# nmichlo/mtg-vision

Measured on AMD Instinct MI355X. Metric: cards/sec end-to-end (detect+embed+top-1 over 100k bank), 640x640, higher is better.
Workload: dtype f32 (products as 3 x f16 MFMA on hi/lo-split operands, f32 accumulate)

## Files before the change

### mtg-vision_amd/csrc/gemm_f32.hip

```cpp
#include "gemm_kernel.h"
#include "gemm_sp.h"
#include "operand_registry.h"

#include <stdlib.h>
#include <string.h>
#include <algorithm>
#include <string>
#include <vector>

namespace mtgv {

GemmArgs linear_args(const float* A, int lda, const float* W, const float* bias, float* Out, int ldo, int M, int N, int K,
                     int act) {
  GemmArgs a;
  a.A = A;
  a.W = W;
  a.Out = Out;
  a.bias = bias;
  a.M = M, a.N = N, a.K = K;
  a.c_total = lda;
  a.Cin = K;
  a.ldo = ldo;
  a.act = act;
  return a;
}

GemmArgs conv_args(const ConvIn& in, const float* W, const float* bias, int cout, int kh, int kw, int stride, int pad,
                   const ConvOut& out, int act) {
  GemmArgs a;
  a.A = in.p, a.a_fmt = in.fmt;
  a.W = W;
  a.bias = bias;
  a.Out = out.p, a.out_fmt = out.fmt;
  a.M = in.n * out.h * out.w, a.N = cout, a.K = kh * kw * in.c;
  a.H = in.h, a.Wd = in.w, a.c_total = in.ct, a.c_off = in.co, a.Cin = in.c;
  a.KH = kh, a.KW = kw, a.stride = stride, a.pad = pad;
  a.OH = out.h, a.OW = out.w, a.OH2 = out.h, a.OW2 = out.w;
  a.ldo = out.ct, a.o_off = out.co;
  a.act = act;
  return a;
}

bool gemm_dispatch_f32(const GemmDev& g, const GemmPlan& pl, bool conv, bool apro, int grid, hipStream_t s) {
  return gemm_dispatch<0>(g, pl, conv, apro, grid, s);
}
bool gemm_dispatch_f16x3(const GemmDev& g, const GemmPlan& pl, bool conv, bool apro, int grid, hipStream_t s);


namespace {
struct GemmProf {
  bool on = false;
  std::vector<hipEvent_t> ev;
  size_t used = 0;
  double flops = 0;
  double bytes = 0;
  long launches = 0;
  struct Rec { int M, N, K, KH, stride, batch, act, apro, grn, topk, tm, tn, bk, sp; double bytes, fill, xflops; };
  std::vector<Rec> recs;
} g_prof;
}

void gemm_profile_enable(bool on) {
  g_prof.on = on;
  g_prof.used = 0;
  g_prof.flops = 0;
  g_prof.bytes = 0;
  g_prof.launches = 0;
  g_prof.recs.clear();
}

void gemm_profile_dump(const char* path) {
  FILE* f = fopen(path, "w");
  MTGV_CHECK(f != nullptr, ERR_RUNTIME, "cannot open %s", path);
  fprintf(f, "idx,M,N,K,KH,stride,batch,act,apro,grn,topk,tm,tn,bk,ms,tflops,bytes,sp,fill,xflops\n");
  for (size_t i = 0; i + 1 < g_prof.used && i / 2 < g_prof.recs.size(); i += 2) {
    HIP_OK(hipEventSynchronize(g_prof.ev[i + 1]));
    float t = 0.f;
    HIP_OK(hipEventElapsedTime(&t, g_prof.ev[i], g_prof.ev[i + 1]));
    const auto& r = g_prof.recs[i / 2];
    const double fl = 2.0 * r.M * r.N * r.K * r.batch + r.xflops;
    fprintf(f, "%zu,%d,%d,%d,%d,%d,%d,%d,%d,%d,%d,%d,%d,%d,%.4f,%.2f,%.0f,%d,%.0f,%.0f\n", i / 2, r.M, r.N, r.K, r.KH, r.stride, r.batch, r.act,
            r.apro, r.grn, r.topk, r.tm, r.tn, r.bk, t, fl / (t * 1e-3) / 1e12, r.bytes, r.sp, r.fill, r.xflops);
  }
  fclose(f);
  gemm_sp_stamps_dump((std::string(path) + ".stamps").c_str());
}

bool gemm_profile_enabled() { return g_prof.on; }
double gemm_profile_bytes() { return g_prof.bytes; }

void gemm_profile_read(double* ms, double* flops, long* launches) {
  double total = 0;
  for (size_t i = 0; i + 1 < g_prof.used; i += 2) {
    HIP_OK(hipEventSynchronize(g_prof.ev[i + 1]));
    float t = 0.f;
    HIP_OK(hipEventElapsedTime(&t, g_prof.ev[i], g_prof.ev[i + 1]));
    total += t;
  }
  if (ms) *ms = total;
  if (flops) *flops = g_prof.flops;
  if (launches) *launches = g_prof.launches;
}

static void prof_begin(const GemmArgs& a, const GemmPlan& pl, hipStream_t s, int sp, double fill, double bytes_override = -1.0,
                       double xflops = 0.0) {
  if (!g_prof.on) return;
  while (g_prof.ev.size() < g_prof.used + 2) {
    hipEvent_t e;
    HIP_OK(hipEventCreate(&e));
    g_prof.ev.push_back(e);
  }
  HIP_OK(hipEventRecord(g_prof.ev[g_prof.used], s));
  const double xfl = (a.W2 != nullptr ? 2.0 * (double)a.M * a.N2 * a.N : 0.0) + xflops;
  g_prof.flops += 2.0 * (double)a.M * a.N * a.K * a.batch + xfl;
  {
    const double a_el = is_conv(a) ? (double)(a.M / (a.OH * a.OW)) * a.H * a.Wd * a.Cin : (double)a.M * a.K;
    const double w_el = (double)a.N * a.K;
    const double o_el = a.topk > 0 ? (double)a.M * ceil_div(a.N, 64) * a.topk * 2
                                   : (a.W2 != nullptr ? (double)a.M * a.N2 + (double)a.N2 * a.N : (double)a.M * a.N);
    const double r_el = a.res != nullptr ? (double)a.M * a.N : 0.0;
    double by = 4.0 * ((a.strideA != 0 || a.batch == 1 ? a.batch : 1) * a_el + (a.strideW != 0 || a.batch == 1 ? a.batch : 1) * w_el +
                       a.batch * (o_el + r_el));
    if (bytes_override >= 0.0) by = bytes_override;
    g_prof.bytes += by;
    g_prof.recs.push_back({a.M, a.N, a.K, a.KH, a.stride, a.batch, a.act, a.a_scale != nullptr, a.grn_part != nullptr, a.topk,
                           pl.tm, pl.tn, pl.bk, sp, by, fill, xfl});
  }
  g_prof.launches += 1;
}
static void prof_end(hipStream_t s) {
  if (!g_prof.on) return;
  HIP_OK(hipEventRecord(g_prof.ev[g_prof.used + 1], s));
  g_prof.used += 2;
}

static int g_prec = -1;

int gemm_precision() {
  if (g_prec < 0) {
    const char* e = getenv("MTGV_GEMM_PREC");
    if (e == nullptr || !*e || !strcmp(e, "f16x3")) g_prec = GEMM_PREC_F16X3;
    else if (!strcmp(e, "f32")) g_prec = GEMM_PREC_F32;
    else MTGV_CHECK(false, ERR_INVALID, "MTGV_GEMM_PREC=%s: expected f32 or f16x3", e);
  }
  return g_prec;
}

void gemm_set_precision(int prec) {
  MTGV_CHECK(prec == GEMM_PREC_F32 || prec == GEMM_PREC_F16X3, ERR_INVALID, "gemm precision %d: 0 (f32) or 1 (f16x3)", prec);
  g_prec = prec;
}

static GemmPlan tile(int tm, int tn, int bk, int M, int N) {
  GemmPlan pl{tm, tn, bk, 0, 0};
  pl.tiles_m = ceil_div(M, pl.bm());
  pl.tiles_n = ceil_div(N, pl.bn());
  return pl;
}

static GemmPlan gemm_plan(int M, int N, int K, bool heavy_epilogue, bool scaled_a) {
  if (const char* e = getenv("MTGV_GEMM_TILE")) {
    int tm = 0, tn = 0, bk = 0;
    if (sscanf(e, "%d,%d,%d", &tm, &tn, &bk) == 3 && (tm == 1 || tm == 2) && tn >= 1 && tn <= 5 && (bk == 16 || bk == 32))
      return tile(tm, tn, bk, M, N);
  }
  const bool split = gemm_precision() == GEMM_PREC_F16X3;
  const double ov = 36.0 + (heavy_epilogue ? 48.0 : 0.0);
  static const double eff_tab[2][3][6] = {
      {{0, 0.88, 0.93, 1.00, 0.80, 0.62},
       {0, 0.85, 0.93, 0.98, 1.00, 0.85},
       {0, 0.80, 0.90, 1.00, 0.85, 0.80}},
      {{0, 0.65, 0.88, 1.00, 0.90, 0.72},
       {0, 0.62, 0.90, 0.97, 1.00, 0.90},
       {0, 0.65, 0.88, 1.00, 0.88, 0.70}}};
  const double* eff = eff_tab[split ? 1 : 0][scaled_a ? 2 : heavy_epilogue ? 1 : 0];
  int best_tn = 1;
  double best = -1;
  const long tiles_m = ceil_div(M, 128);
  for (int tn = 1; tn <= 5; ++tn) {
// ... 29 lines not shown
  if (gemm_sp_topk_layout(a, slots, cols)) return;
  const GemmPlan pl = plan_for(a);
  *slots = pl.tiles_n;
  *cols = pl.bn();
}

size_t gemm_grn_part_floats_max(int M, int N, int hw) {
  size_t mx = 0;
  for (int unit : {32, 64, 128, 256}) {
    const size_t f = (size_t)ceil_div(M, unit) * ((unit - 1) / hw + 2) * N;
    mx = f > mx ? f : mx;
  }
  return mx;
}

static bool ln_fusable(const GemmArgs& a, const GemmPlan& pl) {
  if (!(pl.tm == 1 && pl.tn == 3 && pl.bk == 16 && is_conv(a) && a.N == pl.bn() && a.M % pl.bm() == 0)) return false;
  if (a.batch != 1 || a.act != ACT_NONE || a.res != nullptr || a.a_scale != nullptr || a.grn_part != nullptr || a.topk > 0 ||
      a.crop_boxes != nullptr || a.m_count != nullptr || is_remap(a) || a.out_fmt != 0 || a.a_fmt != 0)
    return false;
  GemmArgs t = a;
  t.ln_w = nullptr;
  return gemm_sp_plan(t).cfg < 0;
}

bool gemm_ln_fusable(const GemmArgs& a) { return ln_fusable(a, plan_for(a)); }

void gemm_launch(const GemmArgs& args, hipStream_t s) {
  GemmArgs a = args;
  const GemmPlan pl = plan_for(a);
  if (a.ln_w != nullptr)
    MTGV_CHECK(a.ln_b != nullptr && ln_fusable(a, pl), ERR_INVALID, "gemm: this launch cannot normalise its rows in the epilogue");
  MTGV_CHECK(a.batch >= 1 && a.batch <= 65535, ERR_INVALID, "gemm: batch=%d", a.batch);
  MTGV_CHECK(a.M > 0 && a.N > 0 && a.K > 0, ERR_INVALID, "gemm: empty problem M=%d N=%d K=%d", a.M, a.N, a.K);
  MTGV_CHECK(a.K % 4 == 0 && a.Cin % 4 == 0 && a.c_total % 4 == 0 && a.c_off % 4 == 0, ERR_INVALID,
             "gemm: K=%d Cin=%d c_total=%d c_off=%d must be multiples of 4", a.K, a.Cin, a.c_total, a.c_off);
  MTGV_CHECK(a.K == a.KH * a.KW * a.Cin, ERR_INVALID, "gemm: K=%d != %d*%d*%d", a.K, a.KH, a.KW, a.Cin);
  MTGV_CHECK(((uintptr_t)a.A % 16) == 0 && ((uintptr_t)a.W % 16) == 0, ERR_INVALID, "gemm: operands must be 16-byte aligned");
  MTGV_CHECK((long)a.M * (long)(a.OH * a.OW > a.hw ? a.OH * a.OW : a.hw) < (1l << 40), ERR_INVALID, "gemm: M too large for fastdiv");
  const bool conv = is_conv(a);
  const bool apro = a.a_scale != nullptr;
  MTGV_CHECK(!(apro && conv), ERR_INVALID, "gemm: GRN prologue only on 1x1");
  MTGV_CHECK(!(apro && a.act != ACT_NONE), ERR_INVALID, "gemm: GRN prologue is only combined with a linear epilogue");
  MTGV_CHECK(a.a_shift == nullptr, ERR_INVALID, "gemm: fold the GRN shift into the bias (fold_shift_into_bias_launch)");
  if (!conv) MTGV_CHECK(a.OH == a.H && a.OW == a.Wd, ERR_INVALID, "gemm: 1x1 geometry mismatch");
  if (apro || a.grn_part) MTGV_CHECK(a.hw > 0 && a.M % a.hw == 0, ERR_INVALID, "gemm: hw=%d must divide M=%d", a.hw, a.M);
  const SpPlan sp = gemm_sp_plan(a);
  if (a.grn_part) {
    const GrnLayout l = grn_layout(a, sp, pl);
    a.segmax = l.segmax;
    a.grn_unit_rows = l.unit_rows;
  }
  if (sp.cfg >= 0) {
    prof_begin(a, pl, s, 1, g_prof.on ? gemm_sp_fill_bytes(a, sp) : 0.0, -1.0, a.xflops);
    gemm_sp_launch(a, sp, s);
    prof_end(s);
    return;
  }

  MTGV_CHECK(a.os_nq == 0, ERR_INVALID, "gemm: the grouped scatter epilogue (os_nq) exists on the LDS-DMA kernel only");
  MTGV_CHECK(a.W2 == nullptr, ERR_INVALID, "gemm: the chained 1x1 exists on the LDS-DMA kernel only");
  MTGV_CHECK(conv_pad_h(a) == a.pad && conv_pad_w(a) == a.pad && a.bias_tab == nullptr, ERR_INVALID,
             "gemm: asymmetric padding and the bias table exist on the LDS-DMA kernel only");
  GemmDev g;
  g.a = a;
  if (gemm_precision() == GEMM_PREC_F16X3 && g.a.W_split == nullptr && a.strideW == 0)
    g.a.W_split = operand_split(a.W, a.K, &g.a.wscale);
  if (gemm_precision() != GEMM_PREC_F16X3) g.a.W_split = nullptr, g.a.wscale = nullptr;
  g.d_ohw = make_fastdiv((uint32_t)(a.OH * a.OW));
  g.d_ow = make_fastdiv((uint32_t)a.OW);
  g.d_cin = make_fastdiv((uint32_t)a.Cin);
  g.d_kwcin = make_fastdiv((uint32_t)(a.KW * a.Cin));
  g.d_hw = make_fastdiv((uint32_t)(a.hw > 0 ? a.hw : 1));
  g.d_cw = make_fastdiv((uint32_t)(a.crop_w > 0 ? a.crop_w : 1));
  g.tiles_m = pl.tiles_m;
  g.tiles_n = pl.tiles_n;
  g.nseg_max = a.hw > 0 ? std::min(pl.bm(), (pl.bm() - 1) / a.hw + 2) : 1;
  {
    const double lim = 4294967296.0 - 65536.0;
    const double a_bytes = (double)a.M * a.c_total * 4.0 + (double)a.c_off * 4.0, w_bytes = (double)a.N * a.K * 4.0;
    const double s_bytes = a.a_scale != nullptr && a.hw > 0 ? (double)(a.M / a.hw) * a.K * 4.0 : 0.0;
    g.off32_ok = a_bytes < lim && w_bytes < lim && s_bytes < lim;
  }
  g.remap = is_remap(a);
  const int grid = pl.tiles_m * pl.tiles_n;

  if (a.topk > 0) {
    MTGV_CHECK(!conv && !apro, ERR_INVALID, "gemm: top-k epilogue needs the 128x64x16 tile");
    MTGV_CHECK(a.cand_s != nullptr && a.cand_i != nullptr && a.topk <= 128, ERR_INVALID, "gemm: bad top-k arguments");
  }
  prof_begin(a, pl, s, 0, (double)grid * a.batch * (pl.bm() + pl.bn()) * a.K * 4.0);
  const bool found = gemm_precision() == GEMM_PREC_F16X3 ? gemm_dispatch_f16x3(g, pl, conv, apro, grid, s)
                                                         : gemm_dispatch_f32(g, pl, conv, apro, grid, s);
  if (found) {
    HIP_OK(hipGetLastError());
    prof_end(s);
    return;
  }
  MTGV_CHECK(false, ERR_INVALID, "gemm: no kernel for tile tm=%d tn=%d bk=%d", pl.tm, pl.tn, pl.bk);
}

__global__ __launch_bounds__(256) void grn_finalize_kernel(const float* __restrict__ part, int bm, int segmax, int hw, int N,
                                                          FastDiv d_hw, FastDiv d_bm, const float* __restrict__ gamma,
                                                          float* __restrict__ scale) {
  extern __shared__ __attribute__((aligned(16))) float sm[];
  float* gx = sm;
  float* red = sm + N;
// ... 59 lines not shown
```

### mtg-vision_amd/csrc/gemm_sp.hip

```cpp
#include "gemm_sp.h"

#include <limits.h>
#include <array>
#include <mutex>
#include <utility>
#include <vector>

#include "gemm_sp_kernel.h"
#include "operand_registry.h"

namespace mtgv {

__global__ __launch_bounds__(256) void sp8_pack_plain_kernel(const float* __restrict__ in, sp_h8* __restrict__ out, long n8) {
  const long i = (long)blockIdx.x * 256 + threadIdx.x;
  if (i >= n8) return;
  sp_h8 hi, lo;
  sp8_split8(*reinterpret_cast<const sp_f4*>(in + i * 8), *reinterpret_cast<const sp_f4*>(in + i * 8 + 4), hi, lo);
  out[2 * i] = hi;
  out[2 * i + 1] = lo;
}

void sp8_pack_plain_launch(const float* in, void* out, long rows, int K, hipStream_t s) {
  MTGV_CHECK(K % 8 == 0, ERR_INVALID, "sp8: K=%d must be a multiple of 8", K);
  const long n8 = rows * (K / 8);
  if (n8 <= 0) return;
  hipLaunchKernelGGL(sp8_pack_plain_kernel, dim3((unsigned)((n8 + 255) / 256)), dim3(256), 0, s, in, (sp_h8*)out, n8);
  HIP_OK(hipGetLastError());
}

const char* sp_zero_page() {
  static char* zero[MTGV_MAX_DEVICES] = {};
  static std::mutex mu;
  const int dev = current_device();
  std::lock_guard<std::mutex> lk(mu);
  if (zero[dev] == nullptr) {
    HIP_OK(hipMalloc((void**)&zero[dev], 256));
    HIP_OK(hipMemset(zero[dev], 0, 256));
  }
  return zero[dev];
}

template <int ID>
void gemm_sp_launch_cfg(const SpDev& g, int amode, hipStream_t s);

namespace {
typedef void (*SpLaunchFn)(const SpDev&, int, hipStream_t);
template <int... ID>
constexpr std::array<SpLaunchFn, sizeof...(ID)> sp_launchers(std::integer_sequence<int, ID...>) {
  return {{&gemm_sp_launch_cfg<ID>...}};
}
const auto kLaunch = sp_launchers(std::make_integer_sequence<int, kSpNumCfg>{});

const double kEff[kSpNumCfg] = {0.93, 1.00, 0.88, 0.80, 0.62, 0.00, 0.00, 0.00};

SpPlan plan_of(int cfg, int M, int N) {
  const SpTile& k = kSpTile[cfg];
  SpPlan pl;
  pl.cfg = cfg, pl.bm = k.bm(), pl.bn = k.bn(), pl.unit_rows = k.wave_rows();
  pl.tiles_m = ceil_div(M, k.bm()), pl.tiles_n = ceil_div(N, k.bn());
  return pl;
}
}

bool window_conv_on() {
  static const bool on = env_int("MTGV_SP_WINDOW", 1) != 0;
  return on;
}

bool window_conv_fits(const GemmArgs& a, const SpPlan& pl) {
  const SpTile& k = kSpTile[pl.cfg];
  if (!(window_conv_on() && a.KH == 3 && a.KW == 3 && a.stride == 1 && conv_pad_h(a) == 1 && conv_pad_w(a) == 1 && a.stride_w <= 0 && a.Cin % k.kps() == 0 &&
        a.OH == a.H && a.OW == a.Wd))
    return false;
  return sp_window_fits(k, a.Wd);
}

static bool n160_instance(const GemmArgs& a) {
  SpPlan p;
  p.cfg = SP_CFG_N160;
  return is_conv(a) && a.a_fmt == 1 && a.W2 == nullptr && a.act == ACT_SILU && a.out_fmt == 1 && a.res == nullptr && a.grn_part == nullptr &&
         !is_remap(a) && a.topk == 0 && window_conv_fits(a, p);
}

bool gemm_sp_active() { return gemm_precision() == GEMM_PREC_F16X3; }

bool gemm_sp_takes_sp8(const float* W, int M, int N, int K, int lda, int c_off) {
  if (!gemm_sp_active()) return false;
  if (K % 8 != 0 || N % 4 != 0 || lda % 8 != 0 || c_off % 8 != 0 || M <= 0) return false;
  return operand_sp8(W, K, nullptr, nullptr);
}

static int chain_cfg(const GemmArgs& a) {
  if (a.W2 == nullptr || a.Out2 == nullptr || !is_conv(a)) return -1;
  if (!(gemm_sp_active() && a.a_fmt == 1 && a.act == ACT_SILU && a.res == nullptr && a.grn_part == nullptr && a.topk == 0 && a.batch == 1 &&
        a.os_nq == 0 && a.a_scale == nullptr && a.ln_w == nullptr))
    return -1;
  if (a.bias_tab == nullptr) {
    if (!(a.os == 1 && a.OH2 == a.OH && a.OW2 == a.OW)) return -1;
  } else {
    if (!(a.bias == nullptr && a.os >= 1 && a.oy >= 0 && a.oy < a.os && a.ox >= 0 && a.ox < a.os && a.OH2 == a.OH * a.os && a.OW2 == a.OW * a.os &&
          ((uintptr_t)a.bias_tab & 15) == 0))
      return -1;
    SpPlan p;
    p.cfg = sp_chain_cfg(a.N);
    if (p.cfg < 0 || window_conv_fits(a, p)) return -1;
  }
  if (sp_chain_cfg(a.N) < 0 || a.N2 <= 0 || a.N2 % 32 != 0 || a.N2 > a.N) return -1;
  if (a.K % 8 != 0 || a.c_total % 8 != 0 || a.c_off % 8 != 0 || a.ldo2 % 4 != 0 || a.o_off2 % 4 != 0 || ((uintptr_t)a.Out2 & 15) != 0) return -1;
  if (a.out_fmt2 == 1 && (a.ldo2 % 8 != 0 || a.o_off2 % 8 != 0)) return -1;
  if (a.stride_w > 0 || a.Cin % 8 != 0) return -1;
  if (!operand_sp8(a.W, a.K, nullptr, nullptr) || !operand_sp8(a.W2, a.N, nullptr, nullptr)) return -1;
  return sp_chain_cfg(a.N);
}
bool gemm_sp_chain_ok(const GemmArgs& a) { return chain_cfg(a) >= 0; }

SpPlan gemm_sp_plan(const GemmArgs& a) {
  SpPlan pl;
  if (a.W2 != nullptr) {
    const int c = chain_cfg(a);
    MTGV_CHECK(c >= 0, ERR_INVALID, "gemm: this launch cannot chain its second layer (M=%d N=%d K=%d N2=%d): ask gemm_sp_chain_ok first", a.M,
               a.N, a.K, a.N2);
    return plan_of(c, a.M, a.N);
  }
  const bool sp8_in = a.a_fmt == 1;
  auto none = [&]() -> SpPlan {
    MTGV_CHECK(!sp8_in && a.out_fmt == 0 && a.res_fmt == 0, ERR_INVALID,
               "gemm: SP8 tensors handed to a launch the SP kernel cannot run (M=%d N=%d K=%d)", a.M, a.N, a.K);
    return pl;
  };
  if (!gemm_sp_active()) return none();
  const bool conv = is_conv(a);
  const bool remap = is_remap(a);
  if (a.batch != 1 || a.crop_boxes != nullptr || a.m_count != nullptr || a.ln_w != nullptr) return none();
  if (a.topk > 0) {
    const SpTile& k1 = kSpTile[SP_CFG_TOPK];
    if (sp8_in || conv || a.K % 8 != 0 || a.c_total % 8 != 0 || a.c_off % 8 != 0 || ((uintptr_t)a.A & 15) != 0 || a.a_scale != nullptr ||
        a.a_mul != 1.0f || a.res != nullptr || a.act != ACT_NONE || a.M < k1.bm() || a.N < k1.bn() || !operand_sp8(a.W, a.K, nullptr, nullptr))
      return none();
    return plan_of(SP_CFG_TOPK, a.M, a.N);
  }
  if (conv && (!sp8_in || a.stride_w > 0 || a.Cin % 8 != 0)) return none();
  if (remap && !sp8_in) return none();
  if (a.K % 8 != 0 || a.c_total % 8 != 0 || a.c_off % 8 != 0 || a.ldo % 4 != 0 || a.o_off % 4 != 0 ||
      (a.res != nullptr && a.ldr % 4 != 0))
    return none();
  if (a.N % 4 != 0 && (a.out_fmt != 0 || a.res != nullptr || a.grn_part != nullptr || remap)) return none();
  if (a.out_fmt == 1 && (a.N % 8 != 0 || a.ldo % 8 != 0 || a.o_off % 8 != 0 || a.grn_part != nullptr)) return none();
  if (a.res != nullptr && a.res_fmt == 1 && (a.ldr % 8 != 0 || a.N % 8 != 0)) return none();
  if (((uintptr_t)a.Out % 16) != 0 || (a.res != nullptr && ((uintptr_t)a.res % 16) != 0)) return none();
  if (sp8_in && a.a_scale != nullptr) return none();
  if (!operand_sp8(a.W, a.K, nullptr, nullptr)) return none();
  if (!sp8_in && (a.N < 64 || a.M < 128)) return none();

  int best = -1;
  double best_cost = 0;
  const int force = env_int("MTGV_SP_CFG", INT_MIN);
  const bool forced = force != INT_MIN;
  if (forced && force >= 0 && force < kSpNumCfg && kSpTile[force].ks == 2 && (force != SP_CFG_N160 || n160_instance(a))) best = force;
  if (best < 0) {
    for (int c = 0; c < kSpNumCfg; ++c) {
      const SpTile& k = kSpTile[c];
      if (kEff[c] <= 0.0) continue;
      if (!sp8_in && a.a_scale != nullptr && sp_ring(k, SP_A_F32_MUL, kSpRing) > kSpTwoPerCu) continue;
      const long tiles = (long)ceil_div(a.M, k.bm()) * ceil_div(a.N, k.bn());
      const double rounds = (double)((tiles + kSpRoundTiles - 1) / kSpRoundTiles);
      const double per_cu = rounds * 2.0 * k.bm() * k.bn();
      const double cost = per_cu / kEff[c];
      if (best < 0 || cost < best_cost) best = c, best_cost = cost;
    }
  }
  if (a.os_nq == kSpTile[SP_CFG_OS_NQ].bn() && !forced) best = SP_CFG_OS_NQ;
  {
    SpPlan p16;
    p16.cfg = SP_CFG_WIN16;
    if (!forced && conv && sp8_in && a.Cin % kSpTile[best].kps() != 0 && a.N <= kSpTile[SP_CFG_WIN16].bn() && window_conv_fits(a, p16))
      best = SP_CFG_WIN16;
  }
  if (!forced && a.N == kSpTile[SP_CFG_N160].bn() && n160_instance(a) && ceil_div(a.M, kSpTile[SP_CFG_N160].bm()) > kSpRoundTiles &&
      env_int("MTGV_DET_HEAD_DIRECT", 1) != 0)
    best = SP_CFG_N160;
  if (best == SP_CFG_TOPK && !conv && sp8_in && a.grn_part != nullptr && a.topk == 0 && a.K >= 256 && a.M >= 12288) best = SP_CFG_PW1_8W;
  return plan_of(best, a.M, a.N);
}

namespace {
struct StampRec { int M, N, K, cfg, amode, act, tiles; long* buf; };
std::vector<StampRec> g_stamps;
bool stamps_on() {
  static const bool on = env_int("MTGV_SP_STAMPS", 0) != 0;
  return on;
}
}

bool gemm_sp_topk_layout(const GemmArgs& a, int* slots, int* cols) {
  const SpPlan pl = gemm_sp_plan(a);
  if (pl.cfg < 0) return false;
  const SpTile& k = kSpTile[pl.cfg];
  *slots = pl.tiles_n * k.wn;
  *cols = k.wave_cols();
  return true;
}

double gemm_sp_fill_bytes(const GemmArgs& a, const SpPlan& pl) {
  const SpTile& k = kSpTile[pl.cfg];
  const double tiles = (double)pl.tiles_m * pl.tiles_n;
  const double b_tile = (double)k.bn() * a.K * 4.0;
  double a_tile = (double)k.bm() * a.K * 4.0;
  if (a.a_fmt == 1 && is_conv(a) && window_conv_fits(a, pl)) a_tile = (double)sp_window_bytes(k, a.Wd) * (a.Cin / k.kps());
  if (a.a_scale != nullptr) a_tile += (double)(a.K / k.kps()) * sp_stage_mul(SP_A_F32_MUL);
  return tiles * (a_tile + b_tile);
}

void gemm_sp_stamps_dump(const char* path) {
  if (g_stamps.empty()) return;
  HIP_OK(hipDeviceSynchronize());
  FILE* f = fopen(path, "wb");
  MTGV_CHECK(f != nullptr, ERR_RUNTIME, "cannot open %s", path);
  std::vector<long> host;
  for (const StampRec& r : g_stamps) {
    const int hdr[8] = {r.M, r.N, r.K, r.cfg, r.amode, r.act, r.tiles, 0};
    fwrite(hdr, sizeof(int), 8, f);
    host.resize((size_t)r.tiles * 8);
    HIP_OK(hipMemcpy(host.data(), r.buf, host.size() * sizeof(long), hipMemcpyDeviceToHost));
    fwrite(host.data(), sizeof(long), host.size(), f);
    HIP_OK(hipFree(r.buf));
  }
  fclose(f);
  g_stamps.clear();
}

int gemm_sp_topk_hi16_range_cols() { return kSpTile[SP_CFG_TOPK].wave_cols(); }
int gemm_sp_topk_hi16_slots(int N) { return ceil_div(N, kSpTile[SP_CFG_TOPK].bn()) * kSpTile[SP_CFG_TOPK].wn; }

// ... 107 lines not shown
```

### mtg-vision_amd/csrc/gemm_sp_cfg.h

```cpp
#pragma once
#include <stddef.h>

namespace mtgv {

struct SpTile {
  int wm, wn, tm, tn, ks;
  constexpr int bm() const { return 32 * tm * wm; }
  constexpr int bn() const { return 32 * tn * wn; }
  constexpr int rb() const { return 64 * ks; }
  constexpr int kps() const { return 16 * ks; }
  constexpr int waves() const { return wm * wn; }
  constexpr int wave_rows() const { return 32 * tm; }
  constexpr int wave_cols() const { return 32 * tn; }
};

constexpr SpTile kSpTile[] = {
    {2, 2, 2, 2, 2},
    {2, 2, 2, 3, 2},
    {4, 1, 1, 3, 2},
    {4, 1, 1, 2, 2},
    {4, 1, 1, 1, 2},
    {4, 2, 1, 3, 2},
    {4, 1, 1, 1, 1},
    {4, 1, 1, 5, 2},
};
constexpr int kSpNumCfg = sizeof(kSpTile) / sizeof(kSpTile[0]);

enum SpCfgId : int {
  SP_CFG_TOPK = 1,
  SP_CFG_OS_NQ = 3,
  SP_CFG_PW1_8W = 5,
  SP_CFG_WIN16 = 6,
  SP_CFG_N160 = 7,
};
static_assert(kSpTile[SP_CFG_PW1_8W].bm() == kSpTile[SP_CFG_TOPK].bm() && kSpTile[SP_CFG_PW1_8W].bn() == kSpTile[SP_CFG_TOPK].bn(),
              "the eight-wave twin covers the same block");
static_assert(kSpTile[SP_CFG_WIN16].ks == 1 && kSpTile[SP_CFG_OS_NQ].bn() == 64 && kSpTile[SP_CFG_N160].bn() == 160, "named configurations");

constexpr bool sp_tile_chains(const SpTile& t) { return t.wn == 1 && t.tm == 1 && t.ks == 2 && t.tn <= 3; }
constexpr int sp_chain_cfg(int N) {
  for (int c = 0; c < kSpNumCfg; ++c)
    if (sp_tile_chains(kSpTile[c]) && kSpTile[c].bn() == N) return c;
  return -1;
}
constexpr int sp_chain_max_n() {
  int n = 0;
  for (int c = 0; c < kSpNumCfg; ++c)
    if (sp_tile_chains(kSpTile[c]) && kSpTile[c].bn() > n) n = kSpTile[c].bn();
  return n;
}

enum SpAMode : int {
  SP_A_SP8 = 0,
  SP_A_REG = 1,
  SP_A_CONV = 2,
  SP_A_F32_MUL = 3,
  SP_A_F32 = 4,
  SP_A_WINDOW = 5,
  SP_A_HI16 = 6,
};
enum SpEpi : int {
  SP_EPI_ARGS = -1,
  SP_EPI_F32 = 0,
  SP_EPI_SP8_OUT = 1,
  SP_EPI_RES_F32 = 2,
  SP_EPI_RES_SP8 = 4,
  SP_EPI_GRN = 8,
  SP_EPI_TOPK = 16,
  SP_EPI_CHAIN = 32,
  SP_EPI_CHAIN_PHASE = 96,
};
constexpr bool sp_epi_chains(int epi) { return epi == SP_EPI_CHAIN || epi == SP_EPI_CHAIN_PHASE; }
constexpr int SP_ACT_ARGS = -1;

constexpr int kSpPiece = 1024;
constexpr int kSpSlab = 32 * 128;
constexpr int kSpRing = 2;
constexpr int kSpDeepRing = 4;
constexpr long kSpRoundTiles = 512;

constexpr int sp_stage_a(const SpTile& t, int amode) { return amode == SP_A_WINDOW ? 0 : t.bm() * t.rb(); }
constexpr int sp_stage_b(const SpTile& t) { return t.bn() * t.rb(); }
constexpr int sp_stage_mul(int amode) { return amode == SP_A_F32_MUL ? kSpPiece : 0; }
constexpr int sp_stage(const SpTile& t, int amode) { return sp_stage_a(t, amode) + sp_stage_b(t) + sp_stage_mul(amode); }
constexpr size_t sp_ring(const SpTile& t, int amode, int nst) { return (size_t)nst * sp_stage(t, amode); }

constexpr int sp_window_px(int bm, int rb, int Wd) {
  const int rpp = kSpPiece / rb;
  return (bm + 2 * Wd + 2 + rpp - 1) / rpp * rpp;
}
constexpr size_t sp_window_bytes(const SpTile& t, int Wd) { return (size_t)sp_window_px(t.bm(), t.rb(), Wd) * t.rb(); }

constexpr int sp_staging_wave(const SpTile& t) { return 32 * 128 * t.tn; }
constexpr int sp_staging_rounds(const SpTile& t, int amode, int nst) {
  return (amode != SP_A_WINDOW && (size_t)t.waves() * sp_staging_wave(t) > sp_ring(t, amode, nst)) ? 2 : 1;
}

constexpr int sp_chain_a2(const SpTile& t) { return t.waves() * kSpSlab; }
constexpr int sp_chain_w2(const SpTile& t) { return t.waves() * kSpSlab * (1 + t.tn); }
constexpr size_t sp_chain_bytes(const SpTile& t, int N2) { return (size_t)sp_chain_w2(t) + (size_t)t.tn * N2 * 128; }

constexpr size_t sp_launch_lds(const SpTile& t, int amode, int epi, int nst, int Wd) {
  size_t lds = sp_ring(t, amode, nst);
  if (amode == SP_A_WINDOW) {
    const size_t win = sp_window_bytes(t, Wd) + lds, stage = (size_t)t.waves() * sp_staging_wave(t);
    lds = win > stage ? win : stage;
  }
  if (sp_epi_chains(epi) && lds < sp_chain_bytes(t, sp_chain_max_n())) lds = sp_chain_bytes(t, sp_chain_max_n());
  return lds;
}

constexpr size_t kSpTwoPerCu = 80 * 1024;
constexpr bool sp_window_fits(const SpTile& t, int Wd) {
  return sp_window_bytes(t, Wd) + sp_ring(t, SP_A_WINDOW, kSpRing) <= kSpTwoPerCu;
}
constexpr int sp_window_ring(const SpTile& t, int Wd, long tiles) {
  return (tiles <= kSpRoundTiles && sp_window_bytes(t, Wd) + sp_ring(t, SP_A_WINDOW, kSpDeepRing) <= kSpTwoPerCu) ? kSpDeepRing : kSpRing;
}
constexpr bool sp_window_ring_deepens(const SpTile& t) { return sp_window_ring(t, 1, 1) == kSpDeepRing; }
static_assert(sp_window_fits(kSpTile[SP_CFG_N160], 80) && !sp_window_ring_deepens(kSpTile[SP_CFG_N160]) &&
                  sp_launch_lds(kSpTile[SP_CFG_N160], SP_A_WINDOW, SP_EPI_SP8_OUT, kSpRing, 80) <= kSpTwoPerCu,
              "the 128 x 160 tile runs two blocks per CU");

}
```

### mtg-vision_amd/csrc/gemm_sp_inst.h

```cpp
#pragma once
#include "gemm_sp_kernel.h"

namespace mtgv {

namespace {
template <int ID, int AMODE, int ACT, int EPI, int NST = kSpRing>
void sp_launch_one(const SpDev& g, hipStream_t s) {
  constexpr SpTile T = kSpTile[ID];
  if constexpr (AMODE == SP_A_WINDOW && NST == kSpRing && sp_window_ring_deepens(T)) {
    if (sp_window_ring(T, g.Wd, (long)g.tiles_m * g.tiles_n) == kSpDeepRing) return sp_launch_one<ID, AMODE, ACT, EPI, kSpDeepRing>(g, s);
  }
  const size_t lds = sp_launch_lds(T, AMODE, EPI, NST, g.Wd);
  constexpr auto kern = gemm_sp_kernel<T.wm, T.wn, T.tm, T.tn, T.ks, NST, AMODE, ACT, EPI>;
  lds_opt_in<kern>(lds, (AMODE == SP_A_WINDOW || sp_epi_chains(EPI)) ? 160 * 1024 : (int)lds);
  hipLaunchKernelGGL(kern, dim3((unsigned)(g.tiles_m * g.tiles_n)), dim3(64 * T.waves()), lds, s, g);
}

template <int ID, int AMODE, int ACT>
void sp_pick(const SpDev& g, int epi, hipStream_t s) {
  MTGV_CHECK(!sp_epi_chains(epi), ERR_RUNTIME, "gemm_sp: no chained-1x1 instance for A mode %d in configuration %d", AMODE, ID);
  sp_launch_one<ID, AMODE, ACT, SP_EPI_ARGS>(g, s);
}
template <int ID, int AMODE, int ACT, int E0, int... ES>
void sp_pick(const SpDev& g, int epi, hipStream_t s) {
  if (epi == E0) sp_launch_one<ID, AMODE, ACT, E0>(g, s);
  else sp_pick<ID, AMODE, ACT, ES...>(g, epi, s);
}

constexpr int SP8_RES = SP_EPI_SP8_OUT | SP_EPI_RES_SP8;

template <int ID, int AMODE>
void sp_pick_conv(const SpDev& g, int epi, hipStream_t s) {
  if (g.act != ACT_SILU) sp_pick<ID, AMODE, SP_ACT_ARGS>(g, epi, s);
  else if constexpr (sp_tile_chains(kSpTile[ID]) && AMODE == SP_A_CONV)
    sp_pick<ID, AMODE, ACT_SILU, SP_EPI_SP8_OUT, SP8_RES, SP_EPI_CHAIN, SP_EPI_CHAIN_PHASE>(g, epi, s);
  else if constexpr (sp_tile_chains(kSpTile[ID])) sp_pick<ID, AMODE, ACT_SILU, SP_EPI_SP8_OUT, SP8_RES, SP_EPI_CHAIN>(g, epi, s);
  else sp_pick<ID, AMODE, ACT_SILU, SP_EPI_SP8_OUT, SP8_RES>(g, epi, s);
}
}

template <int ID>
void gemm_sp_launch_cfg(const SpDev& g, int amode, hipStream_t s);

#if SP_CFG_ID == 7
static_assert(SP_CFG_ID == SP_CFG_N160, "the single-instance configuration");
template <>
void gemm_sp_launch_cfg<SP_CFG_N160>(const SpDev& g, int amode, hipStream_t s) {
  MTGV_CHECK(amode == SP_A_WINDOW && g.act == ACT_SILU && g.topk == 0 && sp_epi_of(g) == SP_EPI_SP8_OUT, ERR_RUNTIME,
             "gemm_sp: configuration %d runs SiLU window convs with SP8 output only (A mode %d, act %d)", (int)SP_CFG_N160, amode, g.act);
  sp_launch_one<SP_CFG_N160, SP_A_WINDOW, ACT_SILU, SP_EPI_SP8_OUT>(g, s);
}
#endif

template <int ID>
void gemm_sp_launch_cfg(const SpDev& g, int amode, hipStream_t s) {
  constexpr SpTile T = kSpTile[ID];
  if (g.topk > 0) {
    if constexpr (ID == SP_CFG_TOPK) {
      MTGV_CHECK((amode == SP_A_F32 || amode == SP_A_HI16) && g.act == ACT_NONE, ERR_INVALID, "gemm_sp: top-k needs aligned f32 queries");
      if (amode == SP_A_HI16) sp_launch_one<ID, SP_A_HI16, ACT_NONE, SP_EPI_TOPK>(g, s);
      else sp_launch_one<ID, SP_A_F32, ACT_NONE, SP_EPI_TOPK>(g, s);
      return;
    } else {
      MTGV_CHECK(false, ERR_INVALID, "gemm_sp: no top-k instance in this configuration");
    }
  }
  const int epi = sp_epi_of(g);
  if constexpr (T.ks != 2) {
    MTGV_CHECK(amode == SP_A_WINDOW || amode == SP_A_CONV, ERR_RUNTIME, "gemm_sp: configuration %d runs convolutions only (A mode %d)", ID, amode);
    if (amode == SP_A_WINDOW) sp_pick_conv<ID, SP_A_WINDOW>(g, epi, s);
    else sp_pick_conv<ID, SP_A_CONV>(g, epi, s);
  } else if (amode == SP_A_SP8) {
    switch (g.act) {
      case ACT_NONE: sp_pick<ID, SP_A_SP8, ACT_NONE, SP_EPI_F32, SP_EPI_SP8_OUT>(g, epi, s); break;
      case ACT_MISH: sp_pick<ID, SP_A_SP8, ACT_MISH, SP_EPI_GRN>(g, epi, s); break;
      case ACT_GELU: sp_pick<ID, SP_A_SP8, ACT_GELU, SP_EPI_GRN>(g, epi, s); break;
      case ACT_SILU: sp_pick<ID, SP_A_SP8, ACT_SILU, SP_EPI_SP8_OUT, SP8_RES>(g, epi, s); break;
      default: sp_pick<ID, SP_A_SP8, SP_ACT_ARGS>(g, epi, s); break;
    }
  } else if (amode == SP_A_REG) {
    if (g.act == ACT_NONE) sp_pick<ID, SP_A_REG, ACT_NONE>(g, epi, s);
    else sp_pick<ID, SP_A_REG, SP_ACT_ARGS>(g, epi, s);
  } else if (amode == SP_A_F32_MUL) {
    if (g.act == ACT_NONE) sp_pick<ID, SP_A_F32_MUL, ACT_NONE, SP_EPI_RES_F32>(g, epi, s);
    else sp_pick<ID, SP_A_F32_MUL, SP_ACT_ARGS>(g, epi, s);
  } else if (amode == SP_A_F32) {
    if (g.act == ACT_NONE) sp_pick<ID, SP_A_F32, ACT_NONE, SP_EPI_F32, SP_EPI_RES_F32>(g, epi, s);
    else sp_pick<ID, SP_A_F32, SP_ACT_ARGS>(g, epi, s);
  } else if (amode == SP_A_WINDOW) {
    sp_pick_conv<ID, SP_A_WINDOW>(g, epi, s);
  } else if (g.act == ACT_NONE) {
    sp_pick<ID, SP_A_CONV, ACT_NONE, SP_EPI_F32, SP_EPI_SP8_OUT>(g, epi, s);
  } else {
    sp_pick_conv<ID, SP_A_CONV>(g, epi, s);
  }
}

#if SP_CFG_ID != 7
template void gemm_sp_launch_cfg<SP_CFG_ID>(const SpDev& g, int amode, hipStream_t s);
#endif

}
```

### mtg-vision_amd/csrc/gemm_sp_kernel.h

```cpp
#pragma once
#include <type_traits>

#include "act.h"
#include "gemm_f32.h"
#include "gemm_sp_cfg.h"
#include "sp8.h"

namespace mtgv {

typedef float spf16 __attribute__((ext_vector_type(16)));

__device__ __forceinline__ spf16 sp_mfma(sp_h8 b, sp_h8 a, spf16 c) {
  return __builtin_amdgcn_mfma_f32_32x32x16_f16(b, a, c, 0, 0, 0);
}

struct SpDev {
  float* cand_s = nullptr;
  int* cand_i = nullptr;
  int topk = 0;
  long* stamps = nullptr;
  const char* A = nullptr;
  long a_rowb = 0;
  long a_offb = 0;
  const char* W = nullptr;
  const float* wscale = nullptr;
  const float* bias = nullptr;
  const void* res = nullptr;
  long ldr = 0;
  int res_fmt = 0;
  float* Out = nullptr;
  long ldo = 0;
  int o_off = 0;
  int out_fmt = 0;
  int M = 0, N = 0, K = 0;
  float* grn_part = nullptr;
  int hw = 1, segmax = 0;
  FastDiv d_hw;
  const float* a_scale = nullptr;
  float a_mul = 1.0f, a_unmul = 1.0f;
  const char* zero = nullptr;
  int off32 = 0;
  int tiles_m = 0, tiles_n = 0;
  int act = 0;
  int H = 1, Wd = 1, Cin = 0, KW = 1, stride = 1, pad = 0, OH = 1, OW = 1;
  FastDiv d_ohw, d_ow, d_cin, d_kw;
  int remap = 0, os = 1, oy = 0, ox = 0, OH2 = 1, OW2 = 1;
  int nq = 0;
  FastDiv d_nq, d_os;
  const char* W2 = nullptr;
  const float* wscale2 = nullptr;
  const float* bias2 = nullptr;
  float* Out2 = nullptr;
  long ldo2 = 0;
  int o_off2 = 0, out_fmt2 = 0, act2 = 0, N2 = 0;
  int pad_w = 0;
  const float* bias_tab = nullptr;
};

inline int sp_epi_of(const SpDev& g) {
  if (g.W2 != nullptr) return g.bias_tab != nullptr ? SP_EPI_CHAIN_PHASE : SP_EPI_CHAIN;
  if (g.remap || g.N % 4 != 0) return SP_EPI_ARGS;
  return (g.out_fmt == 1 ? SP_EPI_SP8_OUT : SP_EPI_F32) | (g.res != nullptr ? (g.res_fmt == 1 ? SP_EPI_RES_SP8 : SP_EPI_RES_F32) : 0) |
         (g.grn_part != nullptr ? SP_EPI_GRN : 0);
}

typedef const __attribute__((address_space(1))) void* sp_gptr;
typedef __attribute__((address_space(3))) void* sp_lptr;

template <int WM, int WN, int TM, int TN, int KS, int NST, int AMODE, int ACT, int EPI>
__global__ __launch_bounds__(64 * WM * WN, (WM * WN == 8 ? 4 : 2)) void gemm_sp_kernel(const SpDev g) {
#pragma clang fp contract(off)
  constexpr SpTile T{WM, WN, TM, TN, KS};
  constexpr int NW = T.waves(), NT = 64 * NW, BM = T.bm(), BN = T.bn();
  constexpr bool GEN = EPI < 0;
  static_assert(TM <= 2, "the epilogue names its slabs");
  static_assert(NST >= 2 && NST <= 4 && (AMODE != SP_A_REG || NST == 2), "ring depth; the register A path is two-deep");
  constexpr int RB = T.rb(), RPP = kSpPiece / RB, SPR = RB / 16;
  constexpr bool AWIN = AMODE == SP_A_WINDOW;
  constexpr bool ADMA = AMODE != SP_A_REG && !AWIN;
  constexpr bool AF32 = AMODE == SP_A_F32_MUL || AMODE == SP_A_F32;
  constexpr bool HI16 = AMODE == SP_A_HI16;
  constexpr int EB = HI16 ? 2 : 4;
  static_assert(!HI16 || (KS == 2 && EPI == SP_EPI_TOPK), "fp16 rows: 128-byte stage rows, top-k epilogue");
  constexpr int SA = sp_stage_a(T, AMODE), SB = sp_stage_b(T), SSC = sp_stage_mul(AMODE), STG = sp_stage(T, AMODE);
  static_assert(AMODE != SP_A_F32_MUL || KS == 2, "the scale image is one DMA piece: 8 images x 32 k");
  constexpr int PA = ADMA ? BM / RPP : 0, PB = BN / RPP, NP = PA + PB;
  constexpr int PPW = (NP + NW - 1) / NW;
  constexpr int CPS = BM * 2 * KS;
  constexpr int CPT = AMODE == SP_A_REG ? CPS / NT : 1;
  static_assert(AMODE != SP_A_REG || CPS % NT == 0, "A chunks must divide over the threads");
  extern __shared__ __attribute__((aligned(1024))) char smem[];

  const int tid = threadIdx.x, lane = tid & 63;
  const int wave = __builtin_amdgcn_readfirstlane(tid >> 6);
  const int wm = wave / WN, wn = wave % WN;
  const int r = lane & 31, h = lane >> 5;

  const long st0 = g.stamps != nullptr ? (long)__builtin_amdgcn_s_memtime() : 0;
  const long rt0 = g.stamps != nullptr ? (long)__builtin_amdgcn_s_memrealtime() : 0;
  long st1 = 0;
  int L;
  {
    const int nwg = gridDim.x, b = blockIdx.x;
    const int q = nwg >> 3, rr = nwg & 7, x = b & 7;
    L = (x < rr ? x * (q + 1) : rr * (q + 1) + (x - rr) * q) + (b >> 3);
  }
  const int tile_n = L % g.tiles_n, tile_m = L / g.tiles_n;
  const int m0 = tile_m * BM, n0 = tile_n * BN;
  const long wrowb = (long)g.K * EB;
  const int kchunks = g.K >> 3;
  constexpr int KPS = 16 * KS * (4 / EB);
  const int nk = (g.K + KPS - 1) / KPS;
  const bool ktail = (g.K % KPS) != 0;

  const char* src[PPW];
  bool tailz[PPW];
  int cslot[PPW], cih0[PPW], ciw0[PPW];
  const char* csrc[PPW];
  const bool conv_fast = AMODE == SP_A_CONV && g.Cin % (16 * KS) == 0;
  uint32_t off32[PPW];
  const bool sfast = g.off32 != 0 && !ktail;
#pragma unroll
  for (int u = 0; u < PPW; ++u) {
// ... 303 lines not shown
            for (int i = 0; i < TM; ++i) {
              const sp_h8 vh = *reinterpret_cast<const sp_h8*>(win + w_off[i] + (((ks * 4 + h * 2 + 0) ^ w_sw[i]) << 4));
              const sp_h8 vl = *reinterpret_cast<const sp_h8*>(win + w_off[i] + (((ks * 4 + h * 2 + 1) ^ w_sw[i]) << 4));
              ah[i] = w_ok[i] ? vh : z8;
              al[i] = w_ok[i] ? vl : z8;
            }
#pragma unroll
            for (int j = 0; j < TN; ++j) {
              bh[j] = *reinterpret_cast<const sp_h8*>(sb + b_off[j] + shi);
              bl[j] = *reinterpret_cast<const sp_h8*>(sb + b_off[j] + slo);
            }
#pragma unroll
            for (int j = 0; j < TN; ++j)
#pragma unroll
              for (int i = 0; i < TM; ++i) {
                acc[i][j] = sp_mfma(bl[j], ah[i], acc[i][j]);
                acc[i][j] = sp_mfma(bh[j], al[i], acc[i][j]);
                acc[i][j] = sp_mfma(bh[j], ah[i], acc[i][j]);
              }
          }
        }
        buf = buf + 1 == NST ? 0 : buf + 1;
        nbuf = nbuf + 1 == NST ? 0 : nbuf + 1;
      }
    }
  } else {
    storeA(0);
    int buf = 0;
    int nbuf = NST - 1;
    for (int t = 0; t < nk; ++t) {
      wait_stage(t + NST - 1 > nk);
      __builtin_amdgcn_s_barrier();
      if (g.stamps != nullptr && t == 0) st1 = (long)__builtin_amdgcn_s_memtime();
      if (t + NST - 1 < nk) {
        issue(t + NST - 1, nbuf);
        loadA(t + 1);
      }
      if (wave_active && HI16) {
        const char* const sb = ring + buf * STG;
  #pragma unroll
        for (int ks = 0; ks < 4; ++ks) {
          const unsigned so = (unsigned)(((ks * 2 + h) ^ swr) << 4);
          sp_h8 ah[TM], bh[TN];
  #pragma unroll
          for (int i = 0; i < TM; ++i) ah[i] = *reinterpret_cast<const sp_h8*>(sb + a_off[i] + so);
  #pragma unroll
          for (int j = 0; j < TN; ++j) bh[j] = *reinterpret_cast<const sp_h8*>(sb + b_off[j] + so);
  #pragma unroll
          for (int j = 0; j < TN; ++j)
  #pragma unroll
            for (int i = 0; i < TM; ++i) acc[i][j] = sp_mfma(bh[j], ah[i], acc[i][j]);
        }
      }
      if constexpr (AF32 && KS == 2 && !HI16) {
        __builtin_amdgcn_sched_barrier(0);
        if (wave_active) {
          const char* const sb = ring + buf * STG;
          sp_f4 xa[2][TM][2], xs[2][TM][2];
          sp_h8 bh[2][TN], bl[2][TN];
  #pragma unroll
          for (int ks = 0; ks < 2; ++ks) {
            const unsigned shi = (unsigned)(((ks * 4 + h * 2 + 0) ^ swr) << 4);
            const unsigned slo = (unsigned)(((ks * 4 + h * 2 + 1) ^ swr) << 4);
  #pragma unroll
            for (int i = 0; i < TM; ++i) {
              xa[ks][i][0] = *reinterpret_cast<const sp_f4*>(sb + a_off[i] + shi);
              xa[ks][i][1] = *reinterpret_cast<const sp_f4*>(sb + a_off[i] + slo);
              if constexpr (AMODE == SP_A_F32_MUL) {
                xs[ks][i][0] = *reinterpret_cast<const sp_f4*>(sb + sc_off[i] + ks * 64);
                xs[ks][i][1] = *reinterpret_cast<const sp_f4*>(sb + sc_off[i] + ks * 64 + 16);
              }
            }
  #pragma unroll
            for (int j = 0; j < TN; ++j) {
              bh[ks][j] = *reinterpret_cast<const sp_h8*>(sb + b_off[j] + shi);
              bl[ks][j] = *reinterpret_cast<const sp_h8*>(sb + b_off[j] + slo);
            }
          }
          if constexpr (AMODE == SP_A_F32_MUL) {
  #pragma unroll
            for (int ks = 0; ks < 2; ++ks)
  #pragma unroll
              for (int i = 0; i < TM; ++i) xa[ks][i][0] = xa[ks][i][0] * xs[ks][i][0], xa[ks][i][1] = xa[ks][i][1] * xs[ks][i][1];
          }
          sp_h8 ah[2][TM], al[2][TM];
  #pragma unroll
          for (int i = 0; i < TM; ++i) sp8_split8_mix(xa[0][i][0], xa[0][i][1], ah[0][i], al[0][i]);
  #pragma unroll
          for (int ks = 0; ks < 2; ++ks) {
            if (ks == 0) {
  #pragma unroll
              for (int i = 0; i < TM; ++i) sp8_split8_mix(xa[1][i][0], xa[1][i][1], ah[1][i], al[1][i]);
            }
  #pragma unroll
            for (int j = 0; j < TN; ++j)
  #pragma unroll
              for (int i = 0; i < TM; ++i) acc[i][j] = sp_mfma(bl[ks][j], ah[ks][i], acc[i][j]);
  #pragma unroll
            for (int j = 0; j < TN; ++j)
  #pragma unroll
              for (int i = 0; i < TM; ++i) acc[i][j] = sp_mfma(bh[ks][j], al[ks][i], acc[i][j]);
  #pragma unroll
            for (int j = 0; j < TN; ++j)
  #pragma unroll
              for (int i = 0; i < TM; ++i) acc[i][j] = sp_mfma(bh[ks][j], ah[ks][i], acc[i][j]);
          }
          constexpr int CV = (AMODE == SP_A_F32_MUL ? 8 : 0) + 16;
// ... 445 lines not shown
```

Baseline: 34060.

## Add six-wave 192x96 tile config for GRN-prologue residual pointwise GEMMs

Adds a new sparse-path GEMM configuration (6 waves, 192x96 block) for 1x1 GEMMs with an f32 GRN-multiplier prologue and an f32 residual epilogue. It is chosen automatically when it needs fewer launch rounds than the otherwise-best tile, which is meant to reduce wave-quantisation tail cost. It sets launch bounds to three blocks per CU for six-wave kernels, excludes the six-wave variant from the specialised f32 KS=2 inner loop so it falls back to the generic path, and extends profiling records with cfg/amode/epi. The generic inner loop may be slower per tile than the specialised one.

```diff
diff --git a/mtg-vision_amd/csrc/gemm_f32.hip b/mtg-vision_amd/csrc/gemm_f32.hip
--- a/mtg-vision_amd/csrc/gemm_f32.hip
+++ b/mtg-vision_amd/csrc/gemm_f32.hip
@@ -55,7 +55,7 @@
   double flops = 0;
   double bytes = 0;
   long launches = 0;
-  struct Rec { int M, N, K, KH, stride, batch, act, apro, grn, topk, tm, tn, bk, sp; double bytes, fill, xflops; };
+  struct Rec { int M, N, K, KH, stride, batch, act, apro, grn, topk, tm, tn, bk, sp; double bytes, fill, xflops; int cfg, amode, epi; };
   std::vector<Rec> recs;
 } g_prof;
 }
@@ -72,15 +72,15 @@
 void gemm_profile_dump(const char* path) {
   FILE* f = fopen(path, "w");
   MTGV_CHECK(f != nullptr, ERR_RUNTIME, "cannot open %s", path);
-  fprintf(f, "idx,M,N,K,KH,stride,batch,act,apro,grn,topk,tm,tn,bk,ms,tflops,bytes,sp,fill,xflops\n");
+  fprintf(f, "idx,M,N,K,KH,stride,batch,act,apro,grn,topk,tm,tn,bk,ms,tflops,bytes,sp,fill,xflops,cfg,amode,epi\n");
   for (size_t i = 0; i + 1 < g_prof.used && i / 2 < g_prof.recs.size(); i += 2) {
     HIP_OK(hipEventSynchronize(g_prof.ev[i + 1]));
     float t = 0.f;
     HIP_OK(hipEventElapsedTime(&t, g_prof.ev[i], g_prof.ev[i + 1]));
     const auto& r = g_prof.recs[i / 2];
     const double fl = 2.0 * r.M * r.N * r.K * r.batch + r.xflops;
-    fprintf(f, "%zu,%d,%d,%d,%d,%d,%d,%d,%d,%d,%d,%d,%d,%d,%.4f,%.2f,%.0f,%d,%.0f,%.0f\n", i / 2, r.M, r.N, r.K, r.KH, r.stride, r.batch, r.act,
-            r.apro, r.grn, r.topk, r.tm, r.tn, r.bk, t, fl / (t * 1e-3) / 1e12, r.bytes, r.sp, r.fill, r.xflops);
+    fprintf(f, "%zu,%d,%d,%d,%d,%d,%d,%d,%d,%d,%d,%d,%d,%d,%.4f,%.2f,%.0f,%d,%.0f,%.0f,%d,%d,%d\n", i / 2, r.M, r.N, r.K, r.KH, r.stride, r.batch, r.act,
+            r.apro, r.grn, r.topk, r.tm, r.tn, r.bk, t, fl / (t * 1e-3) / 1e12, r.bytes, r.sp, r.fill, r.xflops, r.cfg, r.amode, r.epi);
   }
   fclose(f);
   gemm_sp_stamps_dump((std::string(path) + ".stamps").c_str());
@@ -103,7 +103,7 @@
 }
 
 static void prof_begin(const GemmArgs& a, const GemmPlan& pl, hipStream_t s, int sp, double fill, double bytes_override = -1.0,
-                       double xflops = 0.0) {
+                       double xflops = 0.0, const SpPath* path = nullptr) {
   if (!g_prof.on) return;
   while (g_prof.ev.size() < g_prof.used + 2) {
     hipEvent_t e;
@@ -124,7 +124,7 @@
     if (bytes_override >= 0.0) by = bytes_override;
     g_prof.bytes += by;
     g_prof.recs.push_back({a.M, a.N, a.K, a.KH, a.stride, a.batch, a.act, a.a_scale != nullptr, a.grn_part != nullptr, a.topk,
-                           pl.tm, pl.tn, pl.bk, sp, by, fill, xfl});
+                           pl.tm, pl.tn, pl.bk, sp, by, fill, xfl, path ? path->cfg : -1, path ? path->amode : -1, path ? path->epi : -1});
   }
   g_prof.launches += 1;
 }
@@ -260,7 +260,9 @@
     a.grn_unit_rows = l.unit_rows;
   }
   if (sp.cfg >= 0) {
-    prof_begin(a, pl, s, 1, g_prof.on ? gemm_sp_fill_bytes(a, sp) : 0.0, -1.0, a.xflops);
+    SpPath path{-1, -1, -1, 0};
+    if (g_prof.on) path = gemm_sp_path(a, sp);
+    prof_begin(a, pl, s, 1, g_prof.on ? gemm_sp_fill_bytes(a, sp) : 0.0, -1.0, a.xflops, &path);
     gemm_sp_launch(a, sp, s);
     prof_end(s);
     return;
diff --git a/mtg-vision_amd/csrc/gemm_sp.hip b/mtg-vision_amd/csrc/gemm_sp.hip
--- a/mtg-vision_amd/csrc/gemm_sp.hip
+++ b/mtg-vision_amd/csrc/gemm_sp.hip
@@ -51,7 +51,7 @@
 }
 const auto kLaunch = sp_launchers(std::make_integer_sequence<int, kSpNumCfg>{});
 
-const double kEff[kSpNumCfg] = {0.93, 1.00, 0.88, 0.80, 0.62, 0.00, 0.00, 0.00};
+const double kEff[kSpNumCfg] = {0.93, 1.00, 0.88, 0.80, 0.62, 0.00, 0.00, 0.00, 0.00};
 
 SpPlan plan_of(int cfg, int M, int N) {
   const SpTile& k = kSpTile[cfg];
@@ -80,6 +80,15 @@
   p.cfg = SP_CFG_N160;
   return is_conv(a) && a.a_fmt == 1 && a.W2 == nullptr && a.act == ACT_SILU && a.out_fmt == 1 && a.res == nullptr && a.grn_part == nullptr &&
          !is_remap(a) && a.topk == 0 && window_conv_fits(a, p);
+}
+
+static int sp_amode_of(const GemmArgs& a, const SpPlan& pl);
+
+static bool pw2_6w_instance(const GemmArgs& a) {
+  SpPlan p;
+  p.cfg = SP_CFG_PW2_6W;
+  return !is_conv(a) && a.a_fmt == 0 && a.W2 == nullptr && a.a_scale != nullptr && a.act == ACT_NONE && a.out_fmt == 0 && a.res != nullptr &&
+         a.res_fmt == 0 && a.grn_part == nullptr && !is_remap(a) && a.topk == 0 && a.N % 4 == 0 && sp_amode_of(a, p) == SP_A_F32_MUL;
 }
 
 bool gemm_sp_active() { return gemm_precision() == GEMM_PREC_F16X3; }
@@ -156,7 +165,9 @@
   double best_cost = 0;
   const int force = env_int("MTGV_SP_CFG", INT_MIN);
   const bool forced = force != INT_MIN;
-  if (forced && force >= 0 && force < kSpNumCfg && kSpTile[force].ks == 2 && (force != SP_CFG_N160 || n160_instance(a))) best = force;
+  if (forced && force >= 0 && force < kSpNumCfg && kSpTile[force].ks == 2 && (force != SP_CFG_N160 || n160_instance(a)) &&
+      (force != SP_CFG_PW2_6W || pw2_6w_instance(a)))
+    best = force;
   if (best < 0) {
     for (int c = 0; c < kSpNumCfg; ++c) {
       const SpTile& k = kSpTile[c];
@@ -179,6 +190,10 @@
   if (!forced && a.N == kSpTile[SP_CFG_N160].bn() && n160_instance(a) && ceil_div(a.M, kSpTile[SP_CFG_N160].bm()) > kSpRoundTiles &&
       env_int("MTGV_DET_HEAD_DIRECT", 1) != 0)
     best = SP_CFG_N160;
+  if (!forced && pw2_6w_instance(a)) {
+    auto rounds = [&](int c) { return ((long)ceil_div(a.M, kSpTile[c].bm()) * ceil_div(a.N, kSpTile[c].bn()) + kSpRoundTiles - 1) / kSpRoundTiles; };
+    if (rounds(SP_CFG_PW2_6W) < rounds(best)) best = SP_CFG_PW2_6W;
+  }
   if (best == SP_CFG_TOPK && !conv && sp8_in && a.grn_part != nullptr && a.topk == 0 && a.K >= 256 && a.M >= 12288) best = SP_CFG_PW1_8W;
   return plan_of(best, a.M, a.N);
 }
diff --git a/mtg-vision_amd/csrc/gemm_sp_c8.hip b/mtg-vision_amd/csrc/gemm_sp_c8.hip
--- /dev/null
+++ b/mtg-vision_amd/csrc/gemm_sp_c8.hip
@@ -0,0 +1,2 @@
+#define SP_CFG_ID 8
+#include "gemm_sp_inst.h"
diff --git a/mtg-vision_amd/csrc/gemm_sp_cfg.h b/mtg-vision_amd/csrc/gemm_sp_cfg.h
--- a/mtg-vision_amd/csrc/gemm_sp_cfg.h
+++ b/mtg-vision_amd/csrc/gemm_sp_cfg.h
@@ -23,6 +23,7 @@
     {4, 2, 1, 3, 2},
     {4, 1, 1, 1, 1},
     {4, 1, 1, 5, 2},
+    {6, 1, 1, 3, 2},
 };
 constexpr int kSpNumCfg = sizeof(kSpTile) / sizeof(kSpTile[0]);
 
@@ -32,12 +33,16 @@
   SP_CFG_PW1_8W = 5,
   SP_CFG_WIN16 = 6,
   SP_CFG_N160 = 7,
+  SP_CFG_PW2_6W = 8,
 };
 static_assert(kSpTile[SP_CFG_PW1_8W].bm() == kSpTile[SP_CFG_TOPK].bm() && kSpTile[SP_CFG_PW1_8W].bn() == kSpTile[SP_CFG_TOPK].bn(),
               "the eight-wave twin covers the same block");
 static_assert(kSpTile[SP_CFG_WIN16].ks == 1 && kSpTile[SP_CFG_OS_NQ].bn() == 64 && kSpTile[SP_CFG_N160].bn() == 160, "named configurations");
+static_assert(kSpTile[SP_CFG_PW2_6W].waves() == 6 && kSpTile[SP_CFG_PW2_6W].bm() == 192 && kSpTile[SP_CFG_PW2_6W].wave_rows() == kSpTile[2].wave_rows() &&
+                  kSpTile[SP_CFG_PW2_6W].bn() == kSpTile[2].bn(),
+              "the six-wave twin: the 128 x 96 tile's wave tile, two more waves of rows");
 
-constexpr bool sp_tile_chains(const SpTile& t) { return t.wn == 1 && t.tm == 1 && t.ks == 2 && t.tn <= 3; }
+constexpr bool sp_tile_chains(const SpTile& t) { return t.wm == 4 && t.wn == 1 && t.tm == 1 && t.ks == 2 && t.tn <= 3; }
 constexpr int sp_chain_cfg(int N) {
   for (int c = 0; c < kSpNumCfg; ++c)
     if (sp_tile_chains(kSpTile[c]) && kSpTile[c].bn() == N) return c;
@@ -121,5 +126,8 @@
 static_assert(sp_window_fits(kSpTile[SP_CFG_N160], 80) && !sp_window_ring_deepens(kSpTile[SP_CFG_N160]) &&
                   sp_launch_lds(kSpTile[SP_CFG_N160], SP_A_WINDOW, SP_EPI_SP8_OUT, kSpRing, 80) <= kSpTwoPerCu,
               "the 128 x 160 tile runs two blocks per CU");
+static_assert(sp_launch_lds(kSpTile[SP_CFG_PW2_6W], SP_A_F32_MUL, SP_EPI_RES_F32, kSpRing, 1) <= kSpTwoPerCu &&
+                  sp_staging_rounds(kSpTile[SP_CFG_PW2_6W], SP_A_F32_MUL, kSpRing) == 1,
+              "the 192 x 96 tile runs two blocks per CU and stages its epilogue in one round");
 
 }
diff --git a/mtg-vision_amd/csrc/gemm_sp_inst.h b/mtg-vision_amd/csrc/gemm_sp_inst.h
--- a/mtg-vision_amd/csrc/gemm_sp_inst.h
+++ b/mtg-vision_amd/csrc/gemm_sp_inst.h
@@ -50,6 +50,15 @@
              "gemm_sp: configuration %d runs SiLU window convs with SP8 output only (A mode %d, act %d)", (int)SP_CFG_N160, amode, g.act);
   sp_launch_one<SP_CFG_N160, SP_A_WINDOW, ACT_SILU, SP_EPI_SP8_OUT>(g, s);
 }
+#elif SP_CFG_ID == 8
+static_assert(SP_CFG_ID == SP_CFG_PW2_6W, "the single-instance configuration");
+template <>
+void gemm_sp_launch_cfg<SP_CFG_PW2_6W>(const SpDev& g, int amode, hipStream_t s) {
+  MTGV_CHECK(amode == SP_A_F32_MUL && g.act == ACT_NONE && g.topk == 0 && sp_epi_of(g) == SP_EPI_RES_F32, ERR_RUNTIME,
+             "gemm_sp: configuration %d runs f32 rows with multipliers and an f32 residual only (A mode %d, act %d)", (int)SP_CFG_PW2_6W, amode,
+             g.act);
+  sp_launch_one<SP_CFG_PW2_6W, SP_A_F32_MUL, ACT_NONE, SP_EPI_RES_F32>(g, s);
+}
 #endif
 
 template <int ID>
@@ -96,7 +105,7 @@
   }
 }
 
-#if SP_CFG_ID != 7
+#if SP_CFG_ID != 7 && SP_CFG_ID != 8
 template void gemm_sp_launch_cfg<SP_CFG_ID>(const SpDev& g, int amode, hipStream_t s);
 #endif
 
diff --git a/mtg-vision_amd/csrc/gemm_sp_kernel.h b/mtg-vision_amd/csrc/gemm_sp_kernel.h
--- a/mtg-vision_amd/csrc/gemm_sp_kernel.h
+++ b/mtg-vision_amd/csrc/gemm_sp_kernel.h
@@ -68,7 +68,7 @@
 typedef __attribute__((address_space(3))) void* sp_lptr;
 
 template <int WM, int WN, int TM, int TN, int KS, int NST, int AMODE, int ACT, int EPI>
-__global__ __launch_bounds__(64 * WM * WN, (WM * WN == 8 ? 4 : 2)) void gemm_sp_kernel(const SpDev g) {
+__global__ __launch_bounds__(64 * WM * WN, (WM * WN == 8 ? 4 : WM * WN == 6 ? 3 : 2)) void gemm_sp_kernel(const SpDev g) {
 #pragma clang fp contract(off)
   constexpr SpTile T{WM, WN, TM, TN, KS};
   constexpr int NW = T.waves(), NT = 64 * NW, BM = T.bm(), BN = T.bn();
@@ -478,7 +478,7 @@
             for (int i = 0; i < TM; ++i) acc[i][j] = sp_mfma(bh[j], ah[i], acc[i][j]);
         }
       }
-      if constexpr (AF32 && KS == 2 && !HI16) {
+      if constexpr (AF32 && KS == 2 && !HI16 && NW != 6) {
         __builtin_amdgcn_sched_barrier(0);
         if (wave_active) {
           const char* const sb = ring + buf * STG;
```

Result: slower. 33150 (-2.7%).
